# zju3dv/OnePose

Measured on AMD Instinct MI355X. Metric: query_frames_per_sec, higher is better.
Workload: dtype f32

## Files before the change

### onepose_amd/csrc/gatsspg_gemm_kernels.hip

```cpp
#include "gatsspg_epilogue.h"
#include "gatsspg_launch.h"

namespace gatsspg {

template <class T, int PREC = 0>
constexpr size_t smem_bytes() {
    static_assert(PREC >= 0 && PREC <= 2, "fp32, bf16x3 or bf16x6: the fp16 modes run on the kernels of gatsspg_split_kernels.hip");
    size_t b = sizeof(float) * T::SMEM_FLOATS;
    if constexpr (PREC == 1) {
        if (Bf3Layout<T>::SMEM_BYTES > b) b = Bf3Layout<T>::SMEM_BYTES;
    }
    if constexpr (PREC == 2) {
        if (Bf6Layout<T>::SMEM_BYTES > b) b = Bf6Layout<T>::SMEM_BYTES;
    }
    return b;
}
template <class T, int PREC>
constexpr int smem_floats_mainloop() { return (int)(smem_bytes<T, PREC>() / sizeof(float)); }

using QkvTileW8 = GemmTile<128, QKV_BN, 4, 2, false>;

template <class T, int PREC = 0, int BT = 0, int DS = 0, int QF = 0>
__global__ __launch_bounds__(T::THREADS, (PREC >= 2 ? 4 : 1)) void qkv_kv_kernel(const float* __restrict__ Wqkv, const float* __restrict__ bqkv,
                                                            const unsigned short* __restrict__ Whi,
                                                            const unsigned short* __restrict__ Wlo,
                                                            const unsigned short* __restrict__ Wl2,
                                                            const float* __restrict__ Z, float* __restrict__ Qbuf,
                                                            float* __restrict__ kvpart, ColLayout L) {
    static_assert(PREC >= 0 && PREC <= 2, "fp32, bf16x3 or bf16x6 (the fp16 modes: qkv_kv_sp_kernel)");
    extern __shared__ __attribute__((aligned(16))) float smem[];
    int rt, ct;
    if (!xcd_tile_map(6, active_tiles(L), rt, ct)) return;
    ct = global_tile(L, ct);
    const int c0 = ct * T::BN;
    const int ld = L.ld;
    const float* A = Wqkv + (size_t)rt * 128 * D;
    const int tid = threadIdx.x, lane = tid & 63, wave = tid >> 6;
    const int wm = wave / T::WN, wn = wave % T::WN, half = lane >> 5, l31 = lane & 31;
    float bias[T::TM][16];
    float* btab = smem + smem_floats_mainloop<T, PREC>();
    if constexpr (BT) {
        static_assert(T::BM == 128 && T::KS == 1, "half a piece of bias values, one wave group");
        if ((tid >> 6) == 0 && lane < 32) glds16(bqkv + rt * 128 + 4 * lane, btab);
    } else if constexpr (PREC != 2) {
        load_bias16<T>(bqkv + rt * 128, wm, half, bias);
    }
    f32x16 acc[T::TM][T::TN];
    zero_acc(acc);
    if constexpr (PREC == 1) {
        const size_t ro = (size_t)rt * 128 * BK;
        auto ah = [&](int kt) { return Whi + ro + (size_t)kt * 768 * BK; };
        auto alo = [&](int kt) { return Wlo + ro + (size_t)kt * 768 * BK; };
        auto bl = [&](int kt) { return Z + (size_t)kt * BK * ld + c0; };
        gemm_mainloop_bf3<T>(acc, reinterpret_cast<unsigned short*>(smem), D / BK, ah, alo, BK, bl, ld);
    } else if constexpr (PREC == 2) {
        const size_t ro = (size_t)rt * 128 * BK;
        gemm_mainloop_bf6<T>(
            acc, reinterpret_cast<unsigned short*>(smem), D / BK,
            [&](int kt, int pl) { return (pl == 0 ? Whi : pl == 1 ? Wlo : Wl2) + ro + (size_t)kt * 768 * BK; }, BK,
            [&](int kt) { return Z + (size_t)kt * BK * ld + c0; }, ld);
    } else {
        auto al = [&](int kt) { return A + kt * BK; };
        auto bl = [&](int kt) { return Z + (size_t)kt * BK * ld + c0; };
        gemm_mainloop<T, decltype(al), decltype(bl), IdentityCol, NoHooks, QF>(acc, smem, D / BK, al, D, bl, ld);
    }
    if constexpr (BT) read_bias16<T>(btab, wm, half, bias);
    else if constexpr (PREC == 2) load_bias16<T>(bqkv + rt * 128, wm, half, bias);

    if (rt < 2) {
#pragma unroll
        for (int tm = 0; tm < T::TM; ++tm)
#pragma unroll
            for (int r = 0; r < 16; ++r) acc[tm][0][r] = elu1_select(acc[tm][0][r] + bias[tm][r]) + 1.f;
        if constexpr (DS) store_tile_regs<T>(acc, Qbuf + (size_t)rt * 128 * ld + c0, ld, [](int, float v) { return v; });
        else store_tile_via_lds<T>(acc, smem, Qbuf + (size_t)rt * 128 * ld + c0, ld, [](int, float v) { return v; });
        return;
    }
    const int h = rt - 2;
    const TileSeg ts = tile_seg(L, c0, T::BN);
    constexpr int TS = T::BN + 4;
    float* Tl = smem;
    float opmx = 0.f;
#pragma unroll
    for (int tm = 0; tm < T::TM; ++tm)
#pragma unroll
        for (int r = 0; r < 16; ++r) {
            const int row = (wm * T::TM + tm) * 32 + mfma_row(r, half);
            const int col = wn * 32 + l31;
            float v = acc[tm][0][r] + bias[tm][r];
            const float kf = elu1_select(v) + 1.f;
            v = row < 64 ? kf : v;
            v = col >= ts.valid ? 0.f : v;
            opmx = fmaxf(opmx, fabsf(v));
            Tl[row * TS + col] = v;
        }
    {
        static_assert(T::WAVES_MN * T::KS == 8 || (T::WAVES_MN * T::KS == 4 && T::TM == 2), "8 waves: 0..3 hold K_h, 4..7 V_h; 4 waves: 0, 1 K_h, 2, 3 V_h");
#pragma unroll
        for (int o = 32; o > 0; o >>= 1) opmx = fmaxf(opmx, __shfl_xor(opmx, o));
        if (lane == 0) {
            float* mx = kvpart + ((size_t)ct * H + h) * KVP + DH * DH + DH;
            if constexpr (T::WAVES_MN * T::KS == 8) {
                mx[wave] = wave < 4 ? 64.f * opmx : opmx;
            } else {
                mx[wave] = wm == 0 ? 64.f * opmx : 0.f;
                mx[4 + wave] = wm == 0 ? 0.f : opmx;
            }
        }
    }
    __syncthreads();
    if (wave < 4) {
        const int qi = wave >> 1, di = wave & 1;
        f32x16 kv;
#pragma unroll
        for (int r = 0; r < 16; ++r) kv[r] = 0.f;
        const float4* ap = reinterpret_cast<const float4*>(Tl + (di * 32 + l31) * TS + half * 32);
        const float4* bp = reinterpret_cast<const float4*>(Tl + (64 + qi * 32 + l31) * TS + half * 32);
#pragma unroll
        for (int v4 = 0; v4 < 8; ++v4) {
            const float4 a = ap[v4], b = bp[v4];
            kv = __builtin_amdgcn_mfma_f32_32x32x2f32(a.x, b.x, kv, 0, 0, 0);
            kv = __builtin_amdgcn_mfma_f32_32x32x2f32(a.y, b.y, kv, 0, 0, 0);
            kv = __builtin_amdgcn_mfma_f32_32x32x2f32(a.z, b.z, kv, 0, 0, 0);
            kv = __builtin_amdgcn_mfma_f32_32x32x2f32(a.w, b.w, kv, 0, 0, 0);
        }
        float* out = kvpart + ((size_t)ct * H + h) * KVP;
#pragma unroll
        for (int r = 0; r < 16; ++r) {
            const int d = di * 32 + mfma_row(r, half);
            out[d * DH + qi * 32 + l31] = kv[r];
        }
        {
            const int d = tid >> 2, qtr = tid & 3;
            const float* kr = Tl + d * TS + qtr * 16;
            float s = 0.f;
#pragma unroll
            for (int m = 0; m < 16; ++m) s += kr[m];
            s += __shfl_xor(s, 1);
            s += __shfl_xor(s, 2);
            if (qtr == 0) out[DH * DH + d] = s;
        }
    }
}

constexpr int KVP4 = KVP / 4;
static_assert(KVP % 4 == 0, "KV partials are summed as float4");
template <int KVF_RS>
__global__ __launch_bounds__(1024) void kv_final_kernel(const float* __restrict__ kvpart, const float* __restrict__ kv_src,
                                                        float* __restrict__ kvfin, const float* __restrict__ W0,
                                                        float* __restrict__ Mop, unsigned short* __restrict__ Mpl,
                                                        float* __restrict__ ksumT, float* __restrict__ zsc, int* __restrict__ statcnt,
                                                        const float* __restrict__ sc, ColLayout L, int cross, int prec, int abl) {
    __shared__ float4 red[16][64];
    __shared__ float4 kvs[64];
    __shared__ float opsum[16];
    __shared__ float opmax[16];
    constexpr int KVF_ROWS = 512 / KVF_RS;
    if (prec >= 3) fp16_saturate_mode();
    const int tid = threadIdx.x;
    const int el = tid & 63, part = tid >> 6;
    const bool ksum_block = blockIdx.x == 16 * KVF_RS;
    const int db = ksum_block ? 16 : blockIdx.x / KVF_RS, rs = blockIdx.x % KVF_RS;
    const int e4 = min(db * 64 + el, KVP4 - 1);
    const int seg = blockIdx.y / H, h = blockIdx.y % H;
    const int frame = seg >> 1, side = seg & 1;
    if (!((L.side_mask >> side) & 1)) return;
    const int tseg = cross ? (seg ^ 1) : seg;
    const int nsrc = side ? L.n2 : L.n1;
    const int rp = (tid >> 2) & (KVF_ROWS / 2 - 1), qq = tid & 3;
    const int mr = rs * KVF_ROWS + 2 * rp;
    vf4 wv[2][4];
    const bool op_thread = !ksum_block && tid < 2 * KVF_ROWS;
    if (op_thread && !(abl & 4)) {
        const float* wr = W0 + (size_t)mr * 512 + 256 + h * DH + 4 * qq;
#pragma unroll
        for (int e = 0; e < 2; ++e)
#pragma unroll
            for (int i = 0; i < 4; ++i) wv[e][i] = ldg4(wr + e * 512 + 16 * i);
    } else {
#pragma unroll
        for (int e = 0; e < 2; ++e)
#pragma unroll
            for (int i = 0; i < 4; ++i) wv[e][i] = (vf4){1.f, 2.f, 3.f, 4.f};
    }
    const bool cached = kv_src != nullptr && side == 1;
    const float* base = cached ? kv_src + ((size_t)frame * H + h) * KVP
                               : kvpart + ((size_t)((frame * L.np + (side ? L.n1p : 0)) / QKV_BN) * H + h) * KVP;
    const int nt = cached ? 1 : (side ? L.n2p : L.n1p) / QKV_BN;
    const int per = (nt + 15) / 16;
    const int tb = part * per, te = min(nt, tb + per);
    constexpr int MAX4 = (DH * DH + DH) / 4;
    float ksb = 0.f, vmx = 0.f;
    const bool need_bound = prec >= 3 || ksum_block;
    if (need_bound)
    for (int t = tid; t < nt; t += 1024) {
        const float4* mp = reinterpret_cast<const float4*>(base + (size_t)t * H * KVP) + MAX4;
        const float4 a = mp[0], b4 = mp[1];
        ksb += fmaxf(fmaxf(a.x, a.y), fmaxf(a.z, a.w));
        vmx = fmaxf(vmx, fmaxf(fmaxf(b4.x, b4.y), fmaxf(b4.z, b4.w)));
    }
    const bool ismax = e4 >= MAX4;
    float4 s = make_float4(0.f, 0.f, 0.f, 0.f);
    for (int tt = tb; tt < te; tt += 8) {
        float4 x[8];
#pragma unroll
        for (int u = 0; u < 8; ++u)
            x[u] = *reinterpret_cast<const float4*>(base + (size_t)min(tt + u, nt - 1) * H * KVP + 4 * e4);
#pragma unroll
        for (int u = 0; u < 8; ++u)
            if (tt + u < te) {
                s.x = ismax ? fmaxf(s.x, x[u].x) : s.x + x[u].x; s.y = ismax ? fmaxf(s.y, x[u].y) : s.y + x[u].y;
                s.z = ismax ? fmaxf(s.z, x[u].z) : s.z + x[u].z; s.w = ismax ? fmaxf(s.w, x[u].w) : s.w + x[u].w;
            }
    }
    red[part][el] = s;
    if (need_bound) {
#pragma unroll
        for (int o = 32; o > 0; o >>= 1) {
            ksb += __shfl_xor(ksb, o);
            vmx = fmaxf(vmx, __shfl_xor(vmx, o));
        }
        if (el == 0) { opsum[part] = ksb; opmax[part] = vmx; }
    }
    __syncthreads();
    if (need_bound) {
        ksb = opsum[0];
        vmx = opmax[0];
#pragma unroll
        for (int p = 1; p < 16; ++p) {
            ksb += opsum[p];
            vmx = fmaxf(vmx, opmax[p]);
        }
    }
    float mscale = 1.f, zfold = 1.f;
    if (prec >= 3) {
        (void)nsrc;
        const float bound = sc[4 + h] * ksb * vmx;
        int e = 0;
        if (bound > 0.f && bound < 3.0e38f) e = min(max(ilogbf(bound) + 1, -100), 100);
        mscale = __builtin_ldexpf(1.f, 14 - e);
        zfold = sc[1] / mscale;
    }
    if (part == 0) {
        float4 tot = red[0][el];
#pragma unroll
        for (int p = 1; p < 16; ++p) {
            const float4 r = red[p][el];
            tot.x = ismax ? fmaxf(tot.x, r.x) : tot.x + r.x; tot.y = ismax ? fmaxf(tot.y, r.y) : tot.y + r.y;
            tot.z = ismax ? fmaxf(tot.z, r.z) : tot.z + r.z; tot.w = ismax ? fmaxf(tot.w, r.w) : tot.w + r.w;
        }
        kvs[el] = tot;
        if (db * 64 + el < KVP4 && rs == 0) {
            if (e4 == MAX4) tot = make_float4(ksb, 0.f, 0.f, 0.f);
            else if (e4 == MAX4 + 1) tot = make_float4(vmx, 0.f, 0.f, 0.f);
            *reinterpret_cast<float4*>(kvfin + ((size_t)seg * H + h) * KVP + 4 * e4) = tot;
            if (ksum_block) {
                if (el < DH / 4) *reinterpret_cast<float4*>(ksumT + ((size_t)tseg * H + h) * DH + 4 * el) = tot;
                if (el == 0) zsc[tseg * H + h] = zfold;
                if (h == 0 && el < STATCNT_PER_SEG) statcnt[tseg * STATCNT_PER_SEG + el] = 0;
            }
        }
    }
    if (ksum_block) return;
    __syncthreads();
    if (!op_thread) return;
    float acc[2][4] = {{0.f, 0.f, 0.f, 0.f}, {0.f, 0.f, 0.f, 0.f}};
    if (!(abl & 1)) {
#pragma unroll
        for (int i = 0; i < 4; ++i)
#pragma unroll
            for (int j = 0; j < 4; ++j) {
                const float4 k4 = kvs[j * 16 + qq + 4 * i];
#pragma unroll
                for (int e = 0; e < 2; ++e) {
                    acc[e][j] = fmaf(wv[e][i][0], k4.x, acc[e][j]);
                    acc[e][j] = fmaf(wv[e][i][1], k4.y, acc[e][j]);
                    acc[e][j] = fmaf(wv[e][i][2], k4.z, acc[e][j]);
                    acc[e][j] = fmaf(wv[e][i][3], k4.w, acc[e][j]);
                }
            }
    } else {
#pragma unroll
        for (int e = 0; e < 2; ++e)
#pragma unroll
            for (int j = 0; j < 4; ++j) acc[e][j] = wv[e][j][0] + kvs[qq].x;
    }
#pragma unroll
// ... 319 lines not shown
            const size_t R = (size_t)L.b * L.n1p;
            const size_t m0 = (size_t)ts.frame * L.n1p + (c0 - ts.seg_start);
            const float sc = planes_prec >= 3 ? (float)(1 << SCORE_SPLIT_SCALE_LOG2) : 1.f;
#pragma unroll
            for (int idx = tid; idx < 32 * 32; idx += T::THREADS) {
                const int pt = idx >> 5, slab = (idx >> 2) & 7, q = idx & 3;
                const float* v = smem + pt * TS + slab * 32 + q * 8;
                unsigned p0[4], p1[4], p2[4];
#pragma unroll
                for (int e = 0; e < 4; ++e) {
                    if (planes_prec >= 3) { fp16_split2(v[2 * e] * sc, v[2 * e + 1] * sc, p0[e], p1[e]); p2[e] = 0; }
                    else bf16_split3(v[2 * e], v[2 * e + 1], p0[e], p1[e], p2[e]);
                }
                unsigned short* d0 = MDTp + ((size_t)slab * R + m0 + pt) * 32 + q * 8;
                *reinterpret_cast<u32x4*>(d0) = (u32x4){p0[0], p0[1], p0[2], p0[3]};
                *reinterpret_cast<u32x4*>(d0 + R * D) = (u32x4){p1[0], p1[1], p1[2], p1[3]};
                if (planes_prec == 2) *reinterpret_cast<u32x4*>(d0 + 2 * R * D) = (u32x4){p2[0], p2[1], p2[2], p2[3]};
            }
        }
    }
}

using ScoreTileW8 = GemmTile<SC_BM, SC_BN, 4, 2, false>;

template <class T, bool RAW>
__global__ __launch_bounds__(T::THREADS) void score_exp_kernel(const float* __restrict__ MDT, const float* __restrict__ MD,
                                                               float* __restrict__ conf, float* __restrict__ rowpart,
                                                               float* __restrict__ colpart, ColLayout L, float scale) {
    extern __shared__ __attribute__((aligned(16))) float smem[];
    const int nrt = (L.n1p + T::BM - 1) / T::BM, nct = L.n2p / T::BN;
    int rt, ct;
    const int frame = blockIdx.y;
    if (!xcd_tile_map(nrt, nct, rt, ct)) return;
    const int ld = L.ld;
    const float* Ap = MDT + ((size_t)frame * L.n1p + rt * T::BM) * D;
    const float* Bp = MD + (size_t)frame * L.np + L.n1p + ct * T::BN;
    f32x16 acc[T::TM][T::TN];
    zero_acc(acc);
    gemm_mainloop<T>(
        acc, smem, D / BK, [&](int kt) { return Ap + kt * BK; }, D,
        [&](int kt) { return Bp + (size_t)kt * BK * ld; }, ld);
    score_epilogue<T, T::BN + 1, false, RAW, false>(acc, smem, conf, rowpart, colpart, L, frame, rt, ct, nrt, nct, 1.f, scale);
}

using WltTile = GemmTile<64, 64, 2, 2, true>;

__global__ __launch_bounds__(256) void gats_wlt_kernel(const float* __restrict__ W, const float* __restrict__ P,
                                                       float* __restrict__ Z, ColLayout L, int add_h) {
    using T = WltTile;
    extern __shared__ __attribute__((aligned(16))) float smem[];
    int rt, ct;
    const int NT = L.ld / T::BN;
    if (!xcd_tile_map(4, NT, rt, ct)) return;
    const int c0 = ct * T::BN, ld = L.ld;
    const TileSeg ts = tile_seg(L, c0, T::BN);
    if (ts.side == 0) return;
    f32x16 acc[T::TM][T::TN];
    zero_acc(acc);
    gemm_mainloop<T>(
        acc, smem, D / BK, [&](int kt) { return W + (size_t)kt * BK * D + rt * 64; }, D,
        [&](int kt) { return P + (size_t)kt * BK * ld + c0; }, ld);
    const int tid = threadIdx.x, lane = tid & 63, wave = tid >> 6;
    const int wm = wave / T::WN, wn = wave % T::WN, half = lane >> 5, l31 = lane & 31;
#pragma unroll
    for (int r = 0; r < 16; ++r) {
        const int row = rt * 64 + wm * 32 + mfma_row(r, half);
        float* p = Z + (size_t)row * ld + c0 + wn * 32 + l31;
        float v = acc[0][0][r];
        if (add_h) v += *p;
        *p = elu1(v);
    }
}

__global__ __launch_bounds__(1024) void weight_scale_kernel(float* __restrict__ packed) {
    __shared__ float red[1024];
    const int m = blockIdx.x, layer = blockIdx.y;
    float* blk = packed + PW_ATTN + (size_t)layer * AttnW::SIZE;
    float mx = 0.f;
    if (m == 0) {
        for (int e = threadIdx.x; e < 768 * 256; e += 1024) mx = fmaxf(mx, fabsf(blk[AttnW::WQKV + e]));
    } else if (m == 1) {
        for (int e = threadIdx.x; e < 512 * 256; e += 1024) mx = fmaxf(mx, fabsf(blk[AttnW::W0 + (size_t)(e >> 8) * 512 + (e & 255)]));
    } else {
        for (int e = threadIdx.x; e < 256 * 512; e += 1024) mx = fmaxf(mx, fabsf(blk[AttnW::W3 + e]));
    }
    red[threadIdx.x] = mx;
    __syncthreads();
    for (int o = 512; o > 0; o >>= 1) {
        if ((int)threadIdx.x < o) red[threadIdx.x] = fmaxf(red[threadIdx.x], red[threadIdx.x + o]);
        __syncthreads();
    }
    if (threadIdx.x == 0) {
        const float top = red[0];
        int e = 0;
        if (top > 0.f && top < 3.0e38f) e = min(max(13 - ilogbf(top), -40), 60);
        blk[AttnW::SC + m] = __builtin_ldexpf(1.f, e);
        if (m == 0) blk[AttnW::SC + 3] = 1.f;
    }
    if (m == 1) {
        for (int h = 0; h < H; ++h) {
            __syncthreads();
            float l1 = 0.f;
            if (threadIdx.x < 512) {
                const float* wr = blk + AttnW::W0 + (size_t)threadIdx.x * 512 + 256 + h * DH;
                for (int q = 0; q < DH; ++q) l1 += fabsf(wr[q]);
            }
            red[threadIdx.x] = l1;
            __syncthreads();
            for (int o = 512; o > 0; o >>= 1) {
                if ((int)threadIdx.x < o) red[threadIdx.x] = fmaxf(red[threadIdx.x], red[threadIdx.x + o]);
                __syncthreads();
            }
            if (threadIdx.x == 0) blk[AttnW::SC + 4 + h] = red[0];
        }
    }
}

__global__ __launch_bounds__(256) void split_weights_kernel(const float* __restrict__ packed, unsigned short* __restrict__ packedb) {
    fp16_saturate_mode();
    const int layer = blockIdx.y;
    const size_t e = (size_t)blockIdx.x * 256 + threadIdx.x;
    const float* src = packed + PW_ATTN + (size_t)layer * AttnW::SIZE;
    unsigned short* dst = packedb + (size_t)layer * AttnWB::SIZE;
    constexpr size_t NQ = 768 * 256, N0 = 512 * 512, N3 = 256 * 512;
    float x, sx;
    size_t hi, lo, lo2, d, h16, l16;
    auto slab_major = [](size_t i, size_t M, size_t K) { const size_t m = i / K, k = i % K; return ((k >> 5) * M + m) * 32 + (k & 31); };
    if (e < NQ) { x = src[AttnW::WQKV + e]; sx = src[AttnW::SC + 0]; d = slab_major(e, 768, 256); hi = AttnWB::QKV_HI + d; lo = AttnWB::QKV_LO + d; lo2 = AttnWB::QKV_LO2 + d; h16 = AttnWB::QKV_H16 + d; l16 = AttnWB::QKV_L16 + d; }
    else if (e < NQ + N0) { x = src[AttnW::W0 + (e - NQ)]; sx = src[AttnW::SC + 1]; d = slab_major(e - NQ, 512, 512); hi = AttnWB::W0_HI + d; lo = AttnWB::W0_LO + d; lo2 = AttnWB::W0_LO2 + d; h16 = AttnWB::W0_H16 + d; l16 = AttnWB::W0_L16 + d; }
    else if (e < NQ + N0 + N3) { x = src[AttnW::W3 + (e - NQ - N0)]; sx = src[AttnW::SC + 2]; d = slab_major(e - NQ - N0, 256, 512); hi = AttnWB::W3_HI + d; lo = AttnWB::W3_LO + d; lo2 = AttnWB::W3_LO2 + d; h16 = AttnWB::W3_H16 + d; l16 = AttnWB::W3_L16 + d; }
    else return;
    const unsigned h = bf16_rne_bits(x);
    const float r1 = x - __uint_as_float(h << 16);
    const unsigned m = bf16_rne_bits(r1);
    dst[hi] = (unsigned short)h;
    dst[lo] = (unsigned short)m;
    dst[lo2] = (unsigned short)bf16_rne_bits(r1 - __uint_as_float(m << 16));
    unsigned fh, fl;
    fp16_split2(x * sx, 0.f, fh, fl);
    dst[h16] = (unsigned short)(fh & 0xFFFFu);
    dst[l16] = (unsigned short)(fl & 0xFFFFu);
}

void launch_split_weights(float* packed, unsigned short* packedb, hipStream_t s) {
    constexpr size_t N = 768 * 256 + 512 * 512 + 256 * 512;
    hipLaunchKernelGGL(weight_scale_kernel, dim3(3, 8), dim3(1024), 0, s, packed);
    hipLaunchKernelGGL(split_weights_kernel, dim3((unsigned)((N + 255) / 256), 8), dim3(256), 0, s, packed, packedb);
}


constexpr int DIET_MIN_TILES = 64;
constexpr int SMALL_NT3 = 64;
static int diet_min_tiles() { return tuning_knob("DIET_MIN_TILES", DIET_MIN_TILES); }

template <class T, int PREC, int BT = 0, int DS = 0, int QF = 0>
static void launch_qkv_t(const float* Wqkv, const float* bqkv, const unsigned short* wb, const Workspace& w, hipStream_t s,
                         ProfileHook* hk) {
    const int NT = active_tiles(w.L);
    allow_big_lds<qkv_kv_kernel<T, PREC, BT, DS, QF>>();
    GATSSPG_LAUNCH(hk, KID_QKV_KV, s, (qkv_kv_kernel<T, PREC, BT, DS, QF>), dim3(xcd_grid(6, NT)), dim3(T::THREADS), (smem_bytes<T, PREC>() + 512 * BT), s,
                   Wqkv, bqkv, wb ? wb + AttnWB::QKV_HI : nullptr,
                   wb ? wb + AttnWB::QKV_LO : nullptr, wb ? wb + AttnWB::QKV_LO2 : nullptr, w.Z,
                   w.Q, w.kvpart, w.L);
}

void launch_qkv_kv(const float* Wqkv, const float* bqkv, const unsigned short* wb, const Workspace& w, hipStream_t s,
                   ProfileHook* hk) {
    if (w.prec >= 3) {
        launch_qkv_kv_sp(Wqkv - AttnW::WQKV + AttnW::SC, bqkv, wb, w, s, hk);
        return;
    }
    if (w.prec == 1) launch_qkv_t<QkvTileW8, 1>(Wqkv, bqkv, wb, w, s, hk);
    else if (w.prec == 2) launch_qkv_t<QkvTileW8, 2>(Wqkv, bqkv, wb, w, s, hk);
    else if (active_tiles(w.L) > diet_min_tiles()) launch_qkv_t<QkvTileW8, 0, 1, 1, 1>(Wqkv, bqkv, wb, w, s, hk);
    else launch_qkv_t<QkvTileW8, 0, 0, 1>(Wqkv, bqkv, wb, w, s, hk);
}

void launch_kv_final(const float* W0, const Workspace& w, int cross, const float* kv_src, hipStream_t s, ProfileHook* hk) {
    GATSSPG_LAUNCH(hk, KID_KV_FINAL, s, kv_final_kernel<1>, dim3(17, w.nseg * H), dim3(1024), 0, s, w.kvpart, kv_src, w.kvfin, W0, w.Mop, w.Mpl,
                   w.ksumT, w.zsc, w.statcnt, W0 - AttnW::W0 + AttnW::SC, w.L, cross, w.prec, 0);
}

template <class T, int PREC, int BT = 0, int QF = 0>
static void launch_mlp0_t(const float* W0, const float* b0, const unsigned short* wb, const Workspace& w, hipStream_t s,
                          ProfileHook* hk) {
    constexpr int SF = PREC != 0;
    allow_big_lds<mlp0_kernel<T, PREC, BT, QF, SF>>();
    const int NT = active_tiles(w.L) / (T::BN / MLP0_BN);
    GATSSPG_LAUNCH(hk, KID_MLP0, s, (mlp0_kernel<T, PREC, BT, QF, SF>), dim3(xcd_grid(512 / T::BM, NT)), dim3(T::THREADS),
                   (smem_bytes<T, PREC>() + sizeof(float) * AttnFoldHooks::ZP_FLOATS + 512 * BT), s, W0, b0,
                   wb ? wb + AttnWB::W0_HI : nullptr, wb ? wb + AttnWB::W0_LO : nullptr,
                   wb ? wb + AttnWB::W0_LO2 : nullptr, w.Z, w.Q, w.Mop, w.Mpl, w.ksumT, w.U,
                   w.statpart, w.stats, nullptr, w.L, g_trace);
}
template <class T, int PREC, int DS = 0>
static void launch_mlp3_t(const float* W3, const float* b3, const unsigned short* wb, const Workspace& w, hipStream_t s,
                          ProfileHook* hk) {
    allow_big_lds<mlp3_kernel<T, PREC, DS>>();
    const int NT = active_tiles(w.L) / (T::BN / 64);
    GATSSPG_LAUNCH(hk, KID_MLP3, s, (mlp3_kernel<T, PREC, DS>), dim3(xcd_grid(256 / T::BM, NT)), dim3(T::THREADS),
                   (smem_bytes<T, PREC>()), s, W3, b3, wb ? wb + AttnWB::W3_HI : nullptr,
                   wb ? wb + AttnWB::W3_LO : nullptr, wb ? wb + AttnWB::W3_LO2 : nullptr, w.U,
                   w.stats, w.Z, w.L);
}

void launch_mlp(const float* W0, const float* b0, const float* W3, const float* b3, const unsigned short* wb, const Workspace& w,
                hipStream_t s, ProfileHook* hk) {
    static const int small_nt3 = tuning_knob("SMALL_NT3", SMALL_NT3);
    const bool sp = w.prec >= 3;
    const float* sc = W0 - AttnW::W0 + AttnW::SC;
    if (sp) launch_mlp0_sp(sc, b0, wb, w, s, hk);
    else if (w.prec == 1) launch_mlp0_t<Mlp0TileW8, 1>(W0, b0, wb, w, s, hk);
    else if (w.prec == 2) launch_mlp0_t<Mlp0TileW8, 2>(W0, b0, wb, w, s, hk);
    else if (active_tiles(w.L) > diet_min_tiles()) launch_mlp0_t<Mlp0TileW8, 0, 1, 1>(W0, b0, wb, w, s, hk);
    else launch_mlp0_t<Mlp0TileW8, 0>(W0, b0, wb, w, s, hk);
    GATSSPG_LAUNCH(hk, KID_STAT_FINAL, s, stat_final_kernel<MLP0_BN>, dim3(w.nseg, 8), dim3(1024), 0, s, w.statpart, w.stats, w.L);
    if (sp) launch_mlp3_sp(sc, b3, wb, w, s, hk);
    else if (w.prec == 1) launch_mlp3_t<Mlp3TileTallW8, 1>(W3, b3, wb, w, s, hk);
    else if (w.prec == 2) launch_mlp3_t<Mlp3TileTallW8, 2>(W3, b3, wb, w, s, hk);
    else if (active_tiles(w.L) <= small_nt3) launch_mlp3_t<Mlp3TileS, 0>(W3, b3, wb, w, s, hk);
    else launch_mlp3_t<Mlp3TileTallW8, 0, 1>(W3, b3, wb, w, s, hk);
}

void launch_final_proj_norm(const float* Wf, const float* bf, const Workspace& w, hipStream_t s, ProfileHook* hk) {
    allow_big_lds<final_proj_norm_kernel>();
    GATSSPG_LAUNCH(hk, KID_FINAL_PROJ, s, final_proj_norm_kernel, dim3(w.L.ld / FinalTile::BN), dim3(FinalTile::THREADS),
                   (smem_bytes<FinalTile>()), s, Wf, bf, w.Z, w.MD, w.MDT, w.MDTp, score_on_split_loop(w.prec, 0) ? w.prec : 0, w.L);
}

int score_tile_rows() { return SC_BM; }
int score_tile_cols() { return ScoreTileW8::BN; }

template <class T, bool RAW>
static void launch_score_t(const Workspace& w, float* conf, float scale, hipStream_t s, ProfileHook* hk) {
    allow_big_lds<score_exp_kernel<T, RAW>>();
    const int nrt = (w.L.n1p + T::BM - 1) / T::BM;
    GATSSPG_LAUNCH(hk, KID_SCORE_EXP, s, (score_exp_kernel<T, RAW>), dim3(xcd_grid(nrt, w.L.n2p / T::BN), w.L.b), dim3(T::THREADS),
                   (smem_bytes<T>()), s, w.MDT, w.MD, conf, w.rowpart, w.colpart, w.L, scale);
}

bool score_on_split_loop(int prec, int shifted) { return !shifted && (prec == 2 || prec == 4); }

void launch_score_exp(const Workspace& w, float* conf, float scale, int shifted, hipStream_t s, ProfileHook* hk) {
    if (score_on_split_loop(w.prec, shifted)) return launch_score_exp_sp(w, conf, scale, s, hk);
    if (shifted) launch_score_t<ScoreTileW8, true>(w, conf, scale, s, hk);
    else launch_score_t<ScoreTileW8, false>(w, conf, scale, s, hk);
}

void launch_gats_wlt(const float* W, const float* P, const Workspace& w, int add_h, hipStream_t s, ProfileHook* hk) {
    const int NT = w.L.ld / WltTile::BN;
    GATSSPG_LAUNCH(hk, KID_GATS_WLT, s, gats_wlt_kernel, dim3(xcd_grid(4, NT)), dim3(256), (smem_bytes<WltTile>()), s, W, P, w.Z,
                   w.L, add_h);
}

}
```

### onepose_amd/csrc/gemm_f32_mfma.h

```cpp
#pragma once
#include "gatsspg_common.h"

namespace gatsspg {

typedef float f32x16 __attribute__((ext_vector_type(16)));
typedef float vf4 __attribute__((ext_vector_type(4)));
__device__ __forceinline__ vf4 ldg4(const float* p) { return *reinterpret_cast<const vf4*>(p); }
typedef vf4 vf4u __attribute__((aligned(4)));

template <int BM_, int BN_, int WM_, int WN_, bool AKM_, bool BU_ = false, int KS_ = 1>
struct GemmTile {
    static constexpr int BM = BM_, BN = BN_, WM = WM_, WN = WN_, KS = KS_;
    static constexpr bool AKM = AKM_, BU = BU_;
    static constexpr int TM = BM / WM / 32;
    static constexpr int TN = BN / WN / 32;
    static constexpr int A_STRIDE = AKM ? BM : (BK + 4);
    static constexpr int A_FLOATS = AKM ? BK * BM : BM * (BK + 4);
    static constexpr int B_FLOATS = BK * BN;
    static constexpr int STAGE_FLOATS = A_FLOATS + B_FLOATS;
    static constexpr int SMEM_FLOATS = 2 * STAGE_FLOATS;
    static constexpr int WAVES_MN = WM * WN;
    static constexpr int THREADS = 64 * WM * WN * KS;
    static constexpr int A_VEC = BM * BK / 4 / THREADS;
    static constexpr int B_PIECES = BK * BN / 4;
// ... 12 lines not shown
struct IdentityCol {
    __device__ __forceinline__ int operator()(int c) const { return c; }
};
__device__ __forceinline__ vf4 ldg4_off(const float* base, unsigned byte_off) {
    return *reinterpret_cast<const vf4*>(reinterpret_cast<const char*>(base) + byte_off);
}
__device__ __forceinline__ vf4 ldg4u_off(const float* base, unsigned byte_off) {
    return *reinterpret_cast<const vf4u*>(reinterpret_cast<const char*>(base) + byte_off);
}


struct NoHooks {
    static constexpr bool ENABLED = false;
};
template <class T, class ASlab, class BSlab, class XSlabA, class XSlabB, class BXform, bool HAS_AUX,
          class BCol = IdentityCol, class Hooks = NoHooks, int QF = 0>
__device__ __forceinline__ void gemm_mainloop_ex(f32x16 (&acc)[T::TM][T::TN], float* smem, int KT, ASlab a_slab, int lda,
                                                 BSlab b_slab, int ldb, XSlabA x_mean, XSlabB x_rstd, BXform bxform,
                                                 BCol bcol = BCol(), Hooks* hooks = nullptr) {
    constexpr int BM = T::BM, BN = T::BN, TM = T::TM, TN = T::TN;
    if constexpr (Hooks::ENABLED)
        static_assert(BN == 64 && T::THREADS == 512 && TM == 1 && TN == 1 && !T::AKM, "fold hooks: 64-column tile, 8 waves, one MFMA tile per wave");
    const int tid = threadIdx.x;
    const int lane = tid & 63;
    const int wave = tid >> 6;
    const int kg = wave / T::WAVES_MN, wq = wave % T::WAVES_MN;
    const int wm = wq / T::WN, wn = wq % T::WN;
    const int half = lane >> 5, l31 = lane & 31;
    static_assert(T::KS == 1 || !T::AKM, "K split: plain row-major fp32 loop only");

    unsigned a_goff[T::A_VEC], b_goff[T::B_VEC], x_goff[T::B_VEC];
    int a_soff[T::A_VEC], b_soff[T::B_VEC];
#pragma unroll
    for (int p = 0; p < T::A_VEC; ++p) {
        const int idx = p * T::THREADS + tid;
        if constexpr (T::AKM) {
            const int k = idx / (BM / 4), m = (idx % (BM / 4)) * 4;
            a_goff[p] = 4u * (unsigned)(k * lda + m);
            a_soff[p] = k * BM + m;
        } else {
            const int r = idx / (BK / 4), c = (idx % (BK / 4)) * 4;
            a_goff[p] = 4u * (unsigned)(r * lda + c);
            a_soff[p] = r * T::A_STRIDE + c;
        }
    }
#pragma unroll
    for (int p = 0; p < T::B_VEC; ++p) {
        const int idx = (p * T::THREADS + tid) % T::B_PIECES;
        const int k = idx / (BN / 4), c = (idx % (BN / 4)) * 4;
        b_goff[p] = 4u * (unsigned)(k * ldb + bcol(c));
        x_goff[p] = 4u * (unsigned)k;
        b_soff[p] = T::A_FLOATS + k * BN + c;
    }
    int afrag[TM], bfrag[TN];
#pragma unroll
    for (int tm = 0; tm < TM; ++tm)
        afrag[tm] = T::AKM ? (half * 16) * BM + (wm * TM + tm) * 32 + l31 : ((wm * TM + tm) * 32 + l31) * T::A_STRIDE + half * 16;
#pragma unroll
    for (int tn = 0; tn < TN; ++tn) bfrag[tn] = T::A_FLOATS + (half * 16) * BN + (wn * TN + tn) * 32 + l31;

    vf4 ra0[T::A_VEC], rb0[T::B_VEC], ra1[T::A_VEC], rb1[T::B_VEC];
    float2 rx0[T::B_VEC], rx1[T::B_VEC];

    constexpr int NPIECE = T::A_VEC + T::B_VEC;
    auto gload_piece = [&](int kt, int q, vf4(&ra)[T::A_VEC], vf4(&rb)[T::B_VEC], float2(&rx)[T::B_VEC]) {
        if (q < T::A_VEC) {
            ra[q] = ldg4_off(a_slab(kt), a_goff[q]);
        } else {
            const int p = q - T::A_VEC;
            if constexpr (T::BU) rb[p] = ldg4u_off(b_slab(kt), b_goff[p]);
            else rb[p] = ldg4_off(b_slab(kt), b_goff[p]);
            if constexpr (HAS_AUX)
                rx[p] = make_float2(*reinterpret_cast<const float*>(reinterpret_cast<const char*>(x_mean(kt)) + x_goff[p]),
                                    *reinterpret_cast<const float*>(reinterpret_cast<const char*>(x_rstd(kt)) + x_goff[p]));
        }
    };
    auto gload = [&](int kt, vf4(&ra)[T::A_VEC], vf4(&rb)[T::B_VEC], float2(&rx)[T::B_VEC]) {
#pragma unroll
        for (int q = 0; q < NPIECE; ++q) gload_piece(kt, q, ra, rb, rx);
    };
    auto swrite = [&](float* stage, const vf4(&ra)[T::A_VEC], const vf4(&rb)[T::B_VEC], const float2(&rx)[T::B_VEC]) {
#pragma unroll
        for (int p = 0; p < T::A_VEC; ++p) *reinterpret_cast<vf4*>(stage + a_soff[p]) = ra[p];
#pragma unroll
        for (int p = 0; p < T::B_VEC; ++p) {
            vf4 v = rb[p];
            if constexpr (HAS_AUX) bxform(v, rx[p]);
            *reinterpret_cast<vf4*>(stage + b_soff[p]) = v;
        }
    };
    auto read_frags = [&](const float* stage, int h, float (&a)[TM][8], float (&b)[TN][8]) {
#pragma unroll
        for (int tm = 0; tm < TM; ++tm) {
            if constexpr (T::AKM) {
#pragma unroll
                for (int s = 0; s < 8; ++s) a[tm][s] = stage[afrag[tm] + (h * 8 + s) * BM];
            } else {
                const vf4* ap = reinterpret_cast<const vf4*>(stage + afrag[tm] + h * 8);
                const vf4 x = ap[0], y = ap[1];
                a[tm][0] = x[0]; a[tm][1] = x[1]; a[tm][2] = x[2]; a[tm][3] = x[3];
                a[tm][4] = y[0]; a[tm][5] = y[1]; a[tm][6] = y[2]; a[tm][7] = y[3];
            }
        }
#pragma unroll
        for (int tn = 0; tn < TN; ++tn)
#pragma unroll
            for (int s = 0; s < 8; ++s) b[tn][s] = stage[bfrag[tn] + (h * 8 + s) * BN];
    };
    auto mfma4 = [&](const float (&a)[TM][8], const float (&b)[TN][8], int s0, int cnt = 4) {
#pragma unroll
        for (int s = s0; s < s0 + cnt; ++s)
#pragma unroll
            for (int tm = 0; tm < TM; ++tm)
#pragma unroll
                for (int tn = 0; tn < TN; ++tn)
                    acc[tm][tn] = __builtin_amdgcn_mfma_f32_32x32x2f32(a[tm][s], b[tn][s], acc[tm][tn], 0, 0, 0);
    };
    auto step = [&](const float* cur, float* nxt, int kt_cur, int kt_load, vf4(&ra)[T::A_VEC], vf4(&rb)[T::B_VEC],
                    float2(&rx)[T::B_VEC]) {
        float a0[TM][8], b0[TN][8], a1[TM][8], b1[TN][8];
        constexpr int GAPS = 5;
        read_frags(cur, 0, a0, b0);
        __builtin_amdgcn_sched_barrier(0);
        mfma4(a0, b0, 0, 2);
        __builtin_amdgcn_sched_barrier(0);
        read_frags(cur, 1, a1, b1);
        if constexpr (Hooks::ENABLED) {
            if (kt_cur >= Hooks::SPLIT) {
                const float* bq = cur + T::A_FLOATS + hooks->wave * 4 * BN + hooks->lane;
                hooks->partial(kt_cur - Hooks::SPLIT, bq[0], bq[BN], bq[2 * BN], bq[3 * BN]);
            }
        }
        __builtin_amdgcn_sched_barrier(0);
        mfma4(a0, b0, 2, 2);
        __builtin_amdgcn_sched_barrier(0);
        swrite(nxt, ra, rb, rx);
        __builtin_amdgcn_sched_barrier(0);
#pragma unroll
        for (int g = 0; g < 6; ++g) {
            if (g < 2) mfma4(a0, b0, 4 + 2 * g, 2);
            else mfma4(a1, b1, 2 * (g - 2), 2);
            __builtin_amdgcn_sched_barrier(0);
            if (g < GAPS) {
#pragma unroll
                for (int q = 0; q < NPIECE; ++q)
                    if (q % GAPS == g) gload_piece(kt_load, q, ra, rb, rx);
                __builtin_amdgcn_sched_barrier(0);
            }
        }
    };

    auto step_qf = [&](const float* cur, float* nxt, int kt_cur, int kt_load, vf4(&ra)[T::A_VEC], vf4(&rb)[T::B_VEC],
                       float2(&rx)[T::B_VEC]) {
        static_assert(!QF || (TM == 1 && TN == 1 && !T::AKM && T::KS == 1), "quarter fragments: one MFMA tile per wave, row-major A");
        float a0[4], b0[4], a1[4], b1[4];
        auto read_q = [&](int q, float (&a)[4], float (&b)[4]) {
            const vf4 x = *reinterpret_cast<const vf4*>(cur + afrag[0] + q * 4);
            a[0] = x[0]; a[1] = x[1]; a[2] = x[2]; a[3] = x[3];
#pragma unroll
            for (int s = 0; s < 4; ++s) b[s] = cur[bfrag[0] + (q * 4 + s) * BN];
        };
        auto mfma2 = [&](const float (&a)[4], const float (&b)[4], int s0) {
            acc[0][0] = __builtin_amdgcn_mfma_f32_32x32x2f32(a[s0], b[s0], acc[0][0], 0, 0, 0);
            acc[0][0] = __builtin_amdgcn_mfma_f32_32x32x2f32(a[s0 + 1], b[s0 + 1], acc[0][0], 0, 0, 0);
        };
        constexpr int GAPS = 5;
        read_q(0, a0, b0);
        __builtin_amdgcn_sched_barrier(0);
        mfma2(a0, b0, 0);
        __builtin_amdgcn_sched_barrier(0);
        read_q(1, a1, b1);
        if constexpr (Hooks::ENABLED) {
            if (kt_cur >= Hooks::SPLIT) {
                const float* bq = cur + T::A_FLOATS + hooks->wave * 4 * BN + hooks->lane;
                hooks->partial(kt_cur - Hooks::SPLIT, bq[0], bq[BN], bq[2 * BN], bq[3 * BN]);
            }
        }
        __builtin_amdgcn_sched_barrier(0);
        mfma2(a0, b0, 2);
        __builtin_amdgcn_sched_barrier(0);
        swrite(nxt, ra, rb, rx);
        read_q(2, a0, b0);
        __builtin_amdgcn_sched_barrier(0);
#pragma unroll
        for (int g = 0; g < 6; ++g) {
            if (g == 0) mfma2(a1, b1, 0);
            else if (g == 1) mfma2(a1, b1, 2);
            else if (g == 2) mfma2(a0, b0, 0);
            else if (g == 3) mfma2(a0, b0, 2);
            else if (g == 4) mfma2(a1, b1, 0);
            else mfma2(a1, b1, 2);
            __builtin_amdgcn_sched_barrier(0);
            if (g == 1) read_q(3, a1, b1);
            if (g < GAPS) {
#pragma unroll
                for (int q = 0; q < NPIECE; ++q)
                    if (q % GAPS == g) gload_piece(kt_load, q, ra, rb, rx);
                __builtin_amdgcn_sched_barrier(0);
            }
        }
    };

    auto step_ks = [&](const float* cur, float* nxt, int kt_cur, int kt_load, vf4(&ra)[T::A_VEC], vf4(&rb)[T::B_VEC],
                       float2(&rx)[T::B_VEC]) {
        float a0[TM][8], b0[TN][8];
        read_frags(cur, kg, a0, b0);
        if constexpr (Hooks::ENABLED) {
            if (kt_cur >= Hooks::SPLIT) {
                const float* bq = cur + T::A_FLOATS + hooks->wave * 4 * BN + hooks->lane;
                hooks->partial(kt_cur - Hooks::SPLIT, bq[0], bq[BN], bq[2 * BN], bq[3 * BN]);
            }
        }
        __builtin_amdgcn_sched_barrier(0);
        mfma4(a0, b0, 0, 2);
        __builtin_amdgcn_sched_barrier(0);
        swrite(nxt, ra, rb, rx);
        __builtin_amdgcn_sched_barrier(0);
#pragma unroll
        for (int g = 0; g < 3; ++g) {
            mfma4(a0, b0, 2 + 2 * g, 2);
            __builtin_amdgcn_sched_barrier(0);
#pragma unroll
            for (int q = 0; q < NPIECE; ++q)
                if (q % 3 == g) gload_piece(kt_load, q, ra, rb, rx);
            __builtin_amdgcn_sched_barrier(0);
        }
    };

    float* buf0 = smem;
    float* buf1 = smem + T::STAGE_FLOATS;
    const int last = KT - 1;
    gload(0, ra1, rb1, rx1);
    gload(min(1, last), ra0, rb0, rx0);
    swrite(buf0, ra1, rb1, rx1);
    gload(min(2, last), ra1, rb1, rx1);
    __syncthreads();
    for (int i = 0; i < KT; i += 2) {
        if constexpr (T::KS == 2) step_ks(buf0, buf1, i, min(i + 3, last), ra0, rb0, rx0);
        else if constexpr (QF) step_qf(buf0, buf1, i, min(i + 3, last), ra0, rb0, rx0);
        else step(buf0, buf1, i, min(i + 3, last), ra0, rb0, rx0);
        __syncthreads();
        if constexpr (T::KS == 2) step_ks(buf1, buf0, i + 1, min(i + 4, last), ra1, rb1, rx1);
        else if constexpr (QF) step_qf(buf1, buf0, i + 1, min(i + 4, last), ra1, rb1, rx1);
        else step(buf1, buf0, i + 1, min(i + 4, last), ra1, rb1, rx1);
        __syncthreads();
        if constexpr (Hooks::ENABLED) hooks->pair_end(i, acc[0][0]);
    }
}

template <class T>
__device__ __forceinline__ void ksplit_reduce(f32x16 (&acc)[T::TM][T::TN], float* smem) {
    if constexpr (T::KS == 2) {
        static_assert(T::TM * T::TN * T::THREADS * 16 <= T::SMEM_FLOATS, "the partial accumulators must fit the operand buffers");
        const int tid = threadIdx.x, lane = tid & 63, wave = tid >> 6;
        const int kg = wave / T::WAVES_MN, wq = wave % T::WAVES_MN;
#pragma unroll
        for (int tm = 0; tm < T::TM; ++tm)
#pragma unroll
            for (int tn = 0; tn < T::TN; ++tn)
#pragma unroll
                for (int r = 0; r < 16; ++r)
                    smem[((((kg * T::WAVES_MN + wq) * T::TM + tm) * T::TN + tn) * 16 + r) * 64 + lane] = acc[tm][tn][r];
        __syncthreads();
#pragma unroll
        for (int tm = 0; tm < T::TM; ++tm)
#pragma unroll
            for (int tn = 0; tn < T::TN; ++tn)
#pragma unroll
                for (int r = 0; r < 16; ++r) {
                    const float o = smem[(((((kg ^ 1) * T::WAVES_MN + wq) * T::TM + tm) * T::TN + tn) * 16 + r) * 64 + lane];
                    acc[tm][tn][r] = kg ? o + acc[tm][tn][r] : acc[tm][tn][r] + o;
                }
        __syncthreads();
    }
}

typedef __bf16 bf16x8 __attribute__((ext_vector_type(8)));
typedef __bf16 bf16x2 __attribute__((ext_vector_type(2)));
typedef float f32x2 __attribute__((ext_vector_type(2)));
typedef unsigned u32x4 __attribute__((ext_vector_type(4)));
typedef unsigned u32x2 __attribute__((ext_vector_type(2)));

__device__ __forceinline__ unsigned bf16_rne_bits(float x) {
    const unsigned u = __float_as_uint(x);
    return (u + 0x7FFFu + ((u >> 16) & 1u)) >> 16;
}
__device__ __forceinline__ void bf16_split2(float a, float b, unsigned& hi, unsigned& lo) {
    const bf16x2 h = __builtin_convertvector((f32x2){a, b}, bf16x2);
    hi = __builtin_bit_cast(unsigned, h);
    const float ra = a - __uint_as_float(hi << 16), rb = b - __uint_as_float(hi & 0xFFFF0000u);
    lo = __builtin_bit_cast(unsigned, __builtin_convertvector((f32x2){ra, rb}, bf16x2));
}

typedef _Float16 f16x8 __attribute__((ext_vector_type(8)));
typedef _Float16 f16x2 __attribute__((ext_vector_type(2)));
__device__ __forceinline__ void fp16_saturate_mode() { __builtin_amdgcn_s_setreg((0 << 11) | (23 << 6) | 1, 1); }
__device__ __forceinline__ void fp16_split2(float a, float b, unsigned& hi, unsigned& lo) {
    const f16x2 h = __builtin_convertvector((f32x2){a, b}, f16x2);
    hi = __builtin_bit_cast(unsigned, h);
    const f32x2 r = {a - (float)h[0], b - (float)h[1]};
    lo = __builtin_bit_cast(unsigned, __builtin_convertvector(r, f16x2));
}

template <class T>
struct Bf3Layout {
    static constexpr int KS = 40;
    static constexpr int A_PLANE = T::BM * KS, B_PLANE = T::BN * KS;
    static constexpr int STAGE = 2 * A_PLANE + 2 * B_PLANE;
    static constexpr size_t SMEM_BYTES = 2 * (size_t)STAGE * 2;
    static constexpr int A_PIECES = T::BM * 4 * 2 / T::THREADS;
    static constexpr int KPT = BK * T::BN / T::THREADS;
    static_assert(KPT == 4 || KPT == 8, "a thread owns 4 or 8 consecutive k of one column");
    static_assert(A_PIECES >= 1 && ((T::BM * 4) % T::THREADS == 0 || T::THREADS % (T::BM * 4) == 0), "A plane of a piece is static");
    static_assert(T::BN % 64 == 0, "a wave covers 64 consecutive columns of one k group");
};

constexpr int TERMS_BF16X3 = 0, TERMS_FP16X4 = 1;
// ... 429 lines not shown
```

Measured before the change: 1244.

## Add paired-column-tile QKV/KV kernel with heavy/light work units

```diff
diff --git a/onepose_amd/csrc/gatsspg_gemm_kernels.hip b/onepose_amd/csrc/gatsspg_gemm_kernels.hip
--- a/onepose_amd/csrc/gatsspg_gemm_kernels.hip
+++ b/onepose_amd/csrc/gatsspg_gemm_kernels.hip
@@ -133,6 +133,131 @@
         {
             const int d = tid >> 2, qtr = tid & 3;
             const float* kr = Tl + d * TS + qtr * 16;
+            float s = 0.f;
+#pragma unroll
+            for (int m = 0; m < 16; ++m) s += kr[m];
+            s += __shfl_xor(s, 1);
+            s += __shfl_xor(s, 2);
+            if (qtr == 0) out[DH * DH + d] = s;
+        }
+    }
+}
+
+using QkvTilePair = GemmTile<128, 2 * QKV_BN, 2, 4, false>;
+static_assert(CP % (2 * QKV_BN) == 0, "a pair of column tiles never straddles a segment");
+inline bool qkv_pairable(const ColLayout& L) { return ((L.tw_first | L.tw_count | (L.n1p / QKV_BN)) & 1) == 0; }
+inline int qkv_pair_grid(int NP) { return 8 * 64 * ((NP + 63) / 64); }
+__device__ __forceinline__ bool qkv_pair_map(int NP, int& pair, int& unit) {
+    const int g = blockIdx.x;
+    const int xcd = g & 7, slot = g >> 3;
+    const int s = slot & 63, heavy = s < 32, i = s & 31;
+    pair = (((slot >> 6) << 3) + (i >> 2)) * 8 + xcd;
+    unit = heavy ? (i & 3) : 4 + (i & 3);
+    return pair < NP;
+}
+__global__ __launch_bounds__(512, 2) void qkv_kv_pair_kernel(const float* __restrict__ Wqkv, const float* __restrict__ bqkv,
+                                                             const float* __restrict__ Z, float* __restrict__ Qbuf,
+                                                             float* __restrict__ kvpart, ColLayout L) {
+    using TQ = QkvTileW8;
+    using TP = QkvTilePair;
+    static_assert(TQ::THREADS == 512 && TP::THREADS == 512 && TQ::SMEM_FLOATS <= TP::SMEM_FLOATS, "one workgroup shape, the pair tile's LDS");
+    extern __shared__ __attribute__((aligned(16))) float smem[];
+    int pair, unit;
+    if (!qkv_pair_map(active_tiles(L) >> 1, pair, unit)) return;
+    const int ct0 = global_tile(L, 2 * pair);
+    const int ld = L.ld;
+    const int tid = threadIdx.x, lane = tid & 63, wave = tid >> 6;
+    const int half = lane >> 5, l31 = lane & 31;
+    const int rt = unit < 4 ? 2 + unit : (unit & 1);
+    float* btab = smem + TP::SMEM_FLOATS;
+    if (wave == 0 && lane < 32) glds16(bqkv + rt * 128 + 4 * lane, btab);
+    const float* A = Wqkv + (size_t)rt * 128 * D;
+    auto al = [&](int kt) { return A + kt * BK; };
+    if (unit >= 4) {
+        const int c0 = (ct0 + ((unit >> 1) & 1)) * TQ::BN;
+        const int wm = wave / TQ::WN;
+        f32x16 acc[TQ::TM][TQ::TN];
+        zero_acc(acc);
+        auto bl = [&](int kt) { return Z + (size_t)kt * BK * ld + c0; };
+        gemm_mainloop<TQ, decltype(al), decltype(bl), IdentityCol, NoHooks, 1>(acc, smem, D / BK, al, D, bl, ld);
+        float bias[TQ::TM][16];
+        read_bias16<TQ>(btab, wm, half, bias);
+#pragma unroll
+        for (int r = 0; r < 16; ++r) acc[0][0][r] = elu1_select(acc[0][0][r] + bias[0][r]) + 1.f;
+        store_tile_regs<TQ>(acc, Qbuf + (size_t)rt * 128 * ld + c0, ld, [](int, float v) { return v; });
+        return;
+    }
+    const int h = unit;
+    const int c0 = ct0 * QKV_BN;
+    const int wm = wave / TP::WN, wn = wave % TP::WN;
+    f32x16 acc[TP::TM][TP::TN];
+    zero_acc(acc);
+    {
+        auto bl = [&](int kt) { return Z + (size_t)kt * BK * ld + c0; };
+        gemm_mainloop<TP, decltype(al), decltype(bl), IdentityCol, NoHooks, 1>(acc, smem, D / BK, al, D, bl, ld);
+    }
+    float bias[TP::TM][16];
+    read_bias16<TP>(btab, wm, half, bias);
+    const TileSeg ts = tile_seg(L, c0, TP::BN);
+    constexpr int TS = QKV_BN + 4;
+    constexpr int TILE = 128 * TS;
+    static_assert(2 * TILE <= TP::SMEM_FLOATS, "the two K/V tiles re-use the operand buffers");
+    float* Tl = smem + (wn >> 1) * TILE;
+    const int tcol = (wn & 1) * 32 + l31;
+    float opmx[TP::TM];
+#pragma unroll
+    for (int tm = 0; tm < TP::TM; ++tm) {
+        opmx[tm] = 0.f;
+#pragma unroll
+        for (int r = 0; r < 16; ++r) {
+            const int row = (wm * TP::TM + tm) * 32 + mfma_row(r, half);
+            float v = acc[tm][0][r] + bias[tm][r];
+            const float kf = elu1_select(v) + 1.f;
+            v = wm == 0 ? kf : v;
+            v = wn * 32 + l31 >= ts.valid ? 0.f : v;
+            opmx[tm] = fmaxf(opmx[tm], fabsf(v));
+            Tl[row * TS + tcol] = v;
+        }
+    }
+    {
+#pragma unroll
+        for (int tm = 0; tm < TP::TM; ++tm) {
+#pragma unroll
+            for (int o = 32; o > 0; o >>= 1) opmx[tm] = fmaxf(opmx[tm], __shfl_xor(opmx[tm], o));
+        }
+        if (lane == 0) {
+            float* mx = kvpart + ((size_t)(ct0 + (wn >> 1)) * H + h) * KVP + DH * DH + DH;
+#pragma unroll
+            for (int tm = 0; tm < TP::TM; ++tm) mx[(wm * TP::TM + tm) * 2 + (wn & 1)] = wm == 0 ? 64.f * opmx[tm] : opmx[tm];
+        }
+    }
+    __syncthreads();
+    {
+        const int tj = wave >> 2, w4 = wave & 3, t4 = tid & 255;
+        const float* Tj = smem + tj * TILE;
+        const int qi = w4 >> 1, di = w4 & 1;
+        f32x16 kv;
+#pragma unroll
+        for (int r = 0; r < 16; ++r) kv[r] = 0.f;
+        const float4* ap = reinterpret_cast<const float4*>(Tj + (di * 32 + l31) * TS + half * 32);
+        const float4* bp = reinterpret_cast<const float4*>(Tj + (64 + qi * 32 + l31) * TS + half * 32);
+#pragma unroll
+        for (int v4 = 0; v4 < 8; ++v4) {
+            const float4 a = ap[v4], b = bp[v4];
+            kv = __builtin_amdgcn_mfma_f32_32x32x2f32(a.x, b.x, kv, 0, 0, 0);
+            kv = __builtin_amdgcn_mfma_f32_32x32x2f32(a.y, b.y, kv, 0, 0, 0);
+            kv = __builtin_amdgcn_mfma_f32_32x32x2f32(a.z, b.z, kv, 0, 0, 0);
+            kv = __builtin_amdgcn_mfma_f32_32x32x2f32(a.w, b.w, kv, 0, 0, 0);
+        }
+        float* out = kvpart + ((size_t)(ct0 + tj) * H + h) * KVP;
+#pragma unroll
+        for (int r = 0; r < 16; ++r) {
+            const int d = di * 32 + mfma_row(r, half);
+            out[d * DH + qi * 32 + l31] = kv[r];
+        }
+        {
+            const int d = t4 >> 2, qtr = t4 & 3;
+            const float* kr = Tj + d * TS + qtr * 16;
             float s = 0.f;
 #pragma unroll
             for (int m = 0; m < 16; ++m) s += kr[m];
@@ -758,6 +883,12 @@
 constexpr int DIET_MIN_TILES = 64;
 constexpr int SMALL_NT3 = 64;
 static int diet_min_tiles() { return tuning_knob("DIET_MIN_TILES", DIET_MIN_TILES); }
+constexpr int QKV_SLOTS = 512;
+constexpr int QKV_PAIR_MAX_TILES = QKV_SLOTS / 4;
+static bool qkv_takes_pairs(const ColLayout& L) {
+    const int NT = active_tiles(L);
+    return NT > diet_min_tiles() && 6 * NT > QKV_SLOTS && NT <= tuning_knob("QKV_PAIR_MAX_TILES", QKV_PAIR_MAX_TILES) && qkv_pairable(L);
+}
 
 template <class T, int PREC, int BT = 0, int DS = 0, int QF = 0>
 static void launch_qkv_t(const float* Wqkv, const float* bqkv, const unsigned short* wb, const Workspace& w, hipStream_t s,
@@ -770,6 +901,12 @@
                    w.Q, w.kvpart, w.L);
 }
 
+static void launch_qkv_pair(const float* Wqkv, const float* bqkv, const Workspace& w, hipStream_t s, ProfileHook* hk) {
+    allow_big_lds<qkv_kv_pair_kernel>();
+    GATSSPG_LAUNCH(hk, KID_QKV_KV, s, qkv_kv_pair_kernel, dim3(qkv_pair_grid(active_tiles(w.L) / 2)), dim3(QkvTilePair::THREADS),
+                   (smem_bytes<QkvTilePair>() + 512), s, Wqkv, bqkv, w.Z, w.Q, w.kvpart, w.L);
+}
+
 void launch_qkv_kv(const float* Wqkv, const float* bqkv, const unsigned short* wb, const Workspace& w, hipStream_t s,
                    ProfileHook* hk) {
     if (w.prec >= 3) {
@@ -778,6 +915,7 @@
     }
     if (w.prec == 1) launch_qkv_t<QkvTileW8, 1>(Wqkv, bqkv, wb, w, s, hk);
     else if (w.prec == 2) launch_qkv_t<QkvTileW8, 2>(Wqkv, bqkv, wb, w, s, hk);
+    else if (qkv_takes_pairs(w.L)) launch_qkv_pair(Wqkv, bqkv, w, s, hk);
     else if (active_tiles(w.L) > diet_min_tiles()) launch_qkv_t<QkvTileW8, 0, 1, 1, 1>(Wqkv, bqkv, wb, w, s, hk);
     else launch_qkv_t<QkvTileW8, 0, 0, 1>(Wqkv, bqkv, wb, w, s, hk);
 }
diff --git a/onepose_amd/csrc/gemm_f32_mfma.h b/onepose_amd/csrc/gemm_f32_mfma.h
--- a/onepose_amd/csrc/gemm_f32_mfma.h
+++ b/onepose_amd/csrc/gemm_f32_mfma.h
@@ -188,17 +188,27 @@
 
     auto step_qf = [&](const float* cur, float* nxt, int kt_cur, int kt_load, vf4(&ra)[T::A_VEC], vf4(&rb)[T::B_VEC],
                        float2(&rx)[T::B_VEC]) {
-        static_assert(!QF || (TM == 1 && TN == 1 && !T::AKM && T::KS == 1), "quarter fragments: one MFMA tile per wave, row-major A");
-        float a0[4], b0[4], a1[4], b1[4];
-        auto read_q = [&](int q, float (&a)[4], float (&b)[4]) {
-            const vf4 x = *reinterpret_cast<const vf4*>(cur + afrag[0] + q * 4);
-            a[0] = x[0]; a[1] = x[1]; a[2] = x[2]; a[3] = x[3];
-#pragma unroll
-            for (int s = 0; s < 4; ++s) b[s] = cur[bfrag[0] + (q * 4 + s) * BN];
+        static_assert(!QF || (!T::AKM && T::KS == 1), "quarter fragments: row-major A, no K split");
+        float a0[TM][4], b0[TN][4], a1[TM][4], b1[TN][4];
+        auto read_q = [&](int q, float (&a)[TM][4], float (&b)[TN][4]) {
+#pragma unroll
+            for (int tm = 0; tm < TM; ++tm) {
+                const vf4 x = *reinterpret_cast<const vf4*>(cur + afrag[tm] + q * 4);
+                a[tm][0] = x[0]; a[tm][1] = x[1]; a[tm][2] = x[2]; a[tm][3] = x[3];
+            }
+#pragma unroll
+            for (int tn = 0; tn < TN; ++tn)
+#pragma unroll
+                for (int s = 0; s < 4; ++s) b[tn][s] = cur[bfrag[tn] + (q * 4 + s) * BN];
         };
-        auto mfma2 = [&](const float (&a)[4], const float (&b)[4], int s0) {
-            acc[0][0] = __builtin_amdgcn_mfma_f32_32x32x2f32(a[s0], b[s0], acc[0][0], 0, 0, 0);
-            acc[0][0] = __builtin_amdgcn_mfma_f32_32x32x2f32(a[s0 + 1], b[s0 + 1], acc[0][0], 0, 0, 0);
+        auto mfma2 = [&](const float (&a)[TM][4], const float (&b)[TN][4], int s0) {
+#pragma unroll
+            for (int s = s0; s < s0 + 2; ++s)
+#pragma unroll
+                for (int tm = 0; tm < TM; ++tm)
+#pragma unroll
+                    for (int tn = 0; tn < TN; ++tn)
+                        acc[tm][tn] = __builtin_amdgcn_mfma_f32_32x32x2f32(a[tm][s], b[tn][s], acc[tm][tn], 0, 0, 0);
         };
         constexpr int GAPS = 5;
         read_q(0, a0, b0);
```

After: 1230. -1.1%, worse.
